# AniketRajpoot/DeepMusicGeneration

Measured on NVIDIA B200. Metric: generated_tokens_per_sec, higher is better.
Workload: dtype bf16

## Files before the change

deepmusicgeneration_b200/csrc/decode_layer.cu:

```cuda
#include <cuda.h>

#include "attention_decode3.cuh"
#include "kernels.cuh"
#include "launch.cuh"

namespace dmg {
namespace {

constexpr int DL_STAGES = 10;
constexpr int DL_STAGE = 128 * 128;
constexpr int DL_B_BYTES = DL_ROWS * 128;
constexpr int DL_D = 512;
constexpr int DL_XA_BYTES = DL_ROWS * DL_D * 2;
constexpr int DL_HS_KB = 4;
constexpr int DL_HS_BYTES = DL_HS_KB * DL_B_BYTES;
constexpr int DL_OWN = DL_ROWS / DL_CLUSTER;
constexpr int DL_X1_BYTES = DL_OWN * DL_D * 4;
constexpr int DL_MMAW = 2;
constexpr int DL_THREADS = 32 * (1 + DL_MMAW + 8);
constexpr int DL_EPI0 = 32 * (1 + DL_MMAW);
constexpr int DL_EPI = 256;
constexpr int DL_LN_BYTES = 4 * DL_D * 4;
constexpr int DL_SMEM = DL_STAGES * DL_STAGE + DL_XA_BYTES + DL_HS_BYTES + DL_X1_BYTES + DL_LN_BYTES + 512  + 1024 ;
constexpr int DL_TMEM_COLS = 512;
constexpr int DL_CHAIN = DL_ROWS;
static_assert(DL_SMEM <= 227 * 1024, "decode_layer_kernel: shared memory budget");

__device__ __forceinline__ uint64_t dl_desc_sw128(uint32_t smem_addr) {
  return (uint64_t)((smem_addr & 0x3FFFFu) >> 4) | (1ull << 16) | (64ull << 32) | (1ull << 46) | (2ull << 61);
}
__host__ __device__ constexpr uint32_t dl_idesc(int M, int N) {
  return (1u << 4) | (1u << 7) | (1u << 10) | ((uint32_t)(N >> 3) << 17) | ((uint32_t)(M >> 4) << 24);
}
__device__ __forceinline__ uint32_t dl_cluster_ctarank() {
  uint32_t r;
  asm volatile("mov.u32 %0, %%cluster_ctarank;" : "=r"(r));
  return r;
}
__device__ __forceinline__ void dl_arrive() { asm volatile("barrier.cluster.arrive.release;" ::: "memory"); }
__device__ __forceinline__ void dl_wait() { asm volatile("barrier.cluster.wait.acquire;" ::: "memory"); }
__device__ __forceinline__ void dl_fence_async_all() { asm volatile("fence.proxy.async;" ::: "memory"); }
__device__ __forceinline__ void dl_fence_async_smem() { asm volatile("fence.proxy.async.shared::cta;" ::: "memory"); }

__device__ __forceinline__ void tmem_ld_32x16(uint32_t taddr, uint32_t (&r)[16]) {
  asm volatile(
      "tcgen05.ld.sync.aligned.32x32b.x16.b32 {%0,%1,%2,%3,%4,%5,%6,%7,%8,%9,%10,%11,%12,%13,%14,%15}, [%16];"
      : "=r"(r[0]), "=r"(r[1]), "=r"(r[2]), "=r"(r[3]), "=r"(r[4]), "=r"(r[5]), "=r"(r[6]), "=r"(r[7]), "=r"(r[8]),
        "=r"(r[9]), "=r"(r[10]), "=r"(r[11]), "=r"(r[12]), "=r"(r[13]), "=r"(r[14]), "=r"(r[15])
      : "r"(taddr)
      : "memory");
}
__device__ __forceinline__ void dl_spin(uint64_t* bar, uint32_t parity) {
  uint32_t n = 0;
  while (!mbar_try_wait(bar, parity))
    if (++n > (1u << 27)) __trap();
}
__device__ __forceinline__ float4 ldcg4(const float* p) { return __ldcg((const float4*)p); }
__device__ __forceinline__ void dl_mark(unsigned long long* dbg, int role, int mark) {
  if (dbg == nullptr) return;
  unsigned long long t;
  asm volatile("mov.u64 %0, %%globaltimer;" : "=l"(t));
  dbg[role * 16 + mark] = t;
}

__device__ __forceinline__ float dl_gelu(float x) {
  float t;
  asm("tanh.approx.f32 %0, %1;" : "=f"(t) : "f"(0.7978845608028654f * (x + 0.044715f * x * x * x)));
  return 0.5f * x * (1.f + t);
}

__device__ __forceinline__ void dl_layernorm(float (&z)[64], const float* __restrict__ w, const float* __restrict__ b, int t) {
  float s = 0.f;
#pragma unroll
  for (int i = 0; i < 64; i++) s += z[i];
  s += __shfl_xor_sync(0xffffffffu, s, 1); s += __shfl_xor_sync(0xffffffffu, s, 2); s += __shfl_xor_sync(0xffffffffu, s, 4);
  const float mean = s * (1.f / DL_D);
  float q = 0.f;
#pragma unroll
  for (int i = 0; i < 64; i++) { const float c = z[i] - mean; q += c * c; }
  q += __shfl_xor_sync(0xffffffffu, q, 1); q += __shfl_xor_sync(0xffffffffu, q, 2); q += __shfl_xor_sync(0xffffffffu, q, 4);
  const float rstd = rsqrtf(q * (1.f / DL_D) + 1e-5f);
#pragma unroll
  for (int kb = 0; kb < 8; kb++) {
    const int c = 64 * kb + 8 * t;
    const float4 w0 = *(const float4*)(w + c), w1 = *(const float4*)(w + c + 4);
    const float4 b0 = *(const float4*)(b + c), b1 = *(const float4*)(b + c + 4);
    float* v = z + 8 * kb;
    v[0] = (v[0] - mean) * rstd * w0.x + b0.x; v[1] = (v[1] - mean) * rstd * w0.y + b0.y;
    v[2] = (v[2] - mean) * rstd * w0.z + b0.z; v[3] = (v[3] - mean) * rstd * w0.w + b0.w;
    v[4] = (v[4] - mean) * rstd * w1.x + b1.x; v[5] = (v[5] - mean) * rstd * w1.y + b1.y;
    v[6] = (v[6] - mean) * rstd * w1.z + b1.z; v[7] = (v[7] - mean) * rstd * w1.w + b1.w;
  }
}
__device__ __forceinline__ void dl_store_xa(uint8_t* xa_s, const float (&z)[64], int r, int t) {
#pragma unroll
  for (int kb = 0; kb < 8; kb++) {
    const float* v = z + 8 * kb;
    *(uint4*)(xa_s + kb * DL_B_BYTES + r * 128 + ((t ^ (r & 7)) << 4)) =
        make_uint4(pack_bf16x2(v[0], v[1]), pack_bf16x2(v[2], v[3]), pack_bf16x2(v[4], v[5]), pack_bf16x2(v[6], v[7]));
  }
}

__device__ __forceinline__ void dl_gather(uint32_t taddr, int nacc, float (&out)[16]) {
  uint32_t r[16];
  tmem_ld_32x16(taddr, r);
  tmem_ld_wait();
#pragma unroll
  for (int i = 0; i < 16; i++) out[i] = __uint_as_float(r[i]);
  for (int c = 1; c < nacc; c++) {
    tmem_ld_32x16(taddr + c * DL_CHAIN, r);
    tmem_ld_wait();
#pragma unroll
    for (int i = 0; i < 16; i++) out[i] += __uint_as_float(r[i]);
  }
}

__device__ __forceinline__ uint32_t dl_mapa(uint32_t local_addr, uint32_t rank) {
  uint32_t r;
  asm volatile("mapa.shared::cluster.u32 %0, %1, %2;" : "=r"(r) : "r"(local_addr), "r"(rank));
  return r;
}
__device__ __forceinline__ void dl_st_cluster_v4(uint32_t addr, uint4 v) {
  asm volatile("st.shared::cluster.v4.b32 [%0], {%1, %2, %3, %4};" ::"r"(addr), "r"(v.x), "r"(v.y), "r"(v.z), "r"(v.w) : "memory");
}

__device__ __forceinline__ void decode_layer_body(const CUtensorMap& tmAttn, const CUtensorMap& tmWo, const CUtensorMap& tmW1,
                                                  const CUtensorMap& tmW2, const CUtensorMap& tmWq, const DecodeLayerArgs& a_in, int cluster,
                                                  uint8_t* dl_smem) {
  DecodeLayerArgs a = a_in;
  if (cluster != 0 || dl_cluster_ctarank() != 0) a.dbg = nullptr;
  uint8_t* tiles = dl_smem + ((1024u - (smem_u32(dl_smem) & 1023u)) & 1023u);
  uint8_t* xa_s = tiles + DL_STAGES * DL_STAGE;
  uint8_t* hs_s = xa_s + DL_XA_BYTES;
  float* x1_s = (float*)(hs_s + DL_HS_BYTES);
  float* ln_s = x1_s + DL_OWN * DL_D;
  uint64_t* full = (uint64_t*)(ln_s + 4 * DL_D);
  uint64_t* empty = full + DL_STAGES;
  uint64_t* tmem_full = empty + DL_STAGES;
  uint64_t* xa_ready = tmem_full + 4;
  uint64_t* hs_ready = xa_ready + 2;
  uint64_t* attn_full = hs_ready + 1;
  uint32_t* tmem_holder = (uint32_t*)(attn_full + 1);

  const int warp = threadIdx.x >> 5, lane = threadIdx.x & 31;
  const int crank = (int)dl_cluster_ctarank();
  const int row0 = a.row_base + cluster * DL_ROWS;
  const bool body = (a.mode & 1) != 0, next = (a.mode & 2) != 0;
  const int nkb_A = a.HD >> 6, nkb_d = DL_D >> 6;
  constexpr int nB = 2, nC = 4, nD = 2;
  const int fB = a.di / DL_CLUSTER, fD = a.n3 / DL_CLUSTER;
  const int nA_use = body ? nkb_A : 0, nB_use = body ? nB * nkb_d : 0, nC_use = body ? nC * DL_HS_KB : 0, nD_use = next ? nD * nkb_d : 0;
  pdl_launch_dependents();

  if (warp == 0 && lane == 0) {
    tma_prefetch_desc(&tmWo); tma_prefetch_desc(&tmW1); tma_prefetch_desc(&tmW2); tma_prefetch_desc(&tmWq); tma_prefetch_desc(&tmAttn);
  }
  if (warp == 1 && lane == 0) {
    for (int s = 0; s < DL_STAGES; s++) { mbar_init(&full[s], 1); mbar_init(&empty[s], 1); }
    for (int p = 0; p < 4; p++) mbar_init(&tmem_full[p], DL_MMAW);
    mbar_init(&xa_ready[0], DL_EPI); mbar_init(&xa_ready[1], DL_EPI); mbar_init(hs_ready, DL_EPI); mbar_init(attn_full, 1);
    mbar_fence_init();
  }
  if (warp == 1 + DL_MMAW) tmem_alloc<DL_TMEM_COLS>(tmem_holder);
  tc_fence_before();
  __syncthreads();
  tc_fence_after();
  const uint32_t tmem_base = *tmem_holder;

  if (warp == 0) {
    if (lane == 0) dl_mark(a.dbg, 0, 0);
    const int total = nA_use + nB_use + nC_use + nD_use;
    int bar_state = 0;
    const uint64_t w_policy = l2_policy_evict_last();
    for (int r = 0; r < total; r += 8) {
      if (body && bar_state == 0 && r >= nA_use) { dl_arrive(); bar_state = 1; }
      if (body && bar_state == 1 && r + 8 > nA_use + DL_STAGES) { dl_wait(); dl_arrive(); bar_state = 2; }
      if (body && bar_state == 2 && r >= nA_use + nB_use) { dl_wait(); dl_arrive(); bar_state = 3; }
      if (body && bar_state == 3 && r + 8 > nA_use + nB_use + nC_use + DL_STAGES) { dl_wait(); dl_arrive(); bar_state = 4; }
      const int i = r + lane;
      if (lane < 8 && i < total) {
        const int s = i % DL_STAGES;
        if (i >= DL_STAGES) dl_spin(&empty[s], (uint32_t)((i / DL_STAGES) - 1) & 1u);
        uint8_t* dst = tiles + s * DL_STAGE;
        const CUtensorMap* tm; int c0, frow, boxes;
        if (i < nA_use) { tm = &tmWo; c0 = i * 64; frow = 64 * crank; boxes = 1; }
        else if (i < nA_use + nB_use) { const int j = i - nA_use; tm = &tmW1; c0 = (j / nB) * 64; frow = fB * crank + 128 * (j % nB); boxes = 2; }
        else if (i < nA_use + nB_use + nC_use) { const int j = i - nA_use - nB_use; tm = &tmW2; c0 = fB * crank + (j / nC) * 64; frow = 128 * (j % nC); boxes = 2; }
        else { const int j = i - nA_use - nB_use - nC_use; tm = &tmWq; c0 = (j / nD) * 64; frow = fD * crank + 128 * (j % nD); boxes = (j % nD) == 0 ? 2 : 1; }
        mbar_expect_tx(&full[s], (uint32_t)(boxes * 64 * 128));
        tma_load_2d_hint(dst, tm, c0, frow, &full[s], w_policy);
        if (boxes == 2) tma_load_2d_hint(dst + 64 * 128, tm, c0, frow + 64, &full[s], w_policy);
      }
      if (r == 0 && body) {
        pdl_wait();
        if (lane == 0) mbar_expect_tx(attn_full, (uint32_t)(nkb_A * DL_B_BYTES));
        __syncwarp();
        if (lane < nkb_A) tma_load_2d(xa_s + lane * DL_B_BYTES, &tmAttn, lane * 64, row0, attn_full);
      }
      __syncwarp();
    }
    if (lane == 0) dl_mark(a.dbg, 0, 6);
    if (body) {
      if (bar_state == 0) { dl_arrive(); bar_state = 1; }
      if (bar_state == 1) { dl_wait(); dl_arrive(); bar_state = 2; }
      if (bar_state == 2) { dl_wait(); dl_arrive(); bar_state = 3; }
      if (bar_state == 3) { dl_wait(); dl_arrive(); bar_state = 4; }
      dl_wait();
    }
  } else if (warp <= DL_MMAW) {
    int it = 0;
    const int mine = warp - 1;
    const uint32_t xa_addr = smem_u32(xa_s), hs_addr = smem_u32(hs_s), tiles_addr = smem_u32(tiles);
    constexpr uint64_t DHI = (1ull << 16) | (64ull << 32) | (1ull << 46) | (2ull << 61);
    auto kblock = [&](int i, uint32_t col, uint32_t idesc, uint32_t b_addr, int kb, int kbx) {
      if ((i & (DL_MMAW - 1)) != mine) return;
      const int s = i % DL_STAGES;
      dl_spin(&full[s], (uint32_t)(i / DL_STAGES) & 1u);
      tc_fence_after();
      if (elect_one()) {
        const uint64_t da = DHI | (uint64_t)(((tiles_addr + s * DL_STAGE) & 0x3FFFFu) >> 4), db = DHI | (uint64_t)((b_addr & 0x3FFFFu) >> 4);
        const uint32_t d = tmem_base + col + (uint32_t)(((kb & kbx) << 2) * DL_CHAIN);
#pragma unroll
        for (int l = 0; l < 4; l++)
          umma_bf16(d + (uint32_t)(l * DL_CHAIN), da + (uint64_t)(2 * l), db + (uint64_t)(2 * l), idesc, kb > kbx ? 1u : 0u);
        umma_commit(&empty[s]);
      }
      __syncwarp();
    };
    constexpr uint32_t ID64 = dl_idesc(64, DL_ROWS), ID128 = dl_idesc(128, DL_ROWS);
    if (lane == 0 && mine == 0) dl_mark(a.dbg, 1, 0);
    if (body) {
      {
        dl_spin(attn_full, 0);
        tc_fence_after();
        for (int kb = 0; kb < nkb_A; kb++) kblock(it++, 0, ID64, xa_addr + kb * DL_B_BYTES, kb, 1);
        if (elect_one()) {
          dl_mark(a.dbg, 1, 1);
          umma_commit(&tmem_full[0]);
        }
      }
      __syncwarp();
      dl_arrive();
      dl_wait();
      dl_arrive();
      {
        dl_spin(&xa_ready[0], 0);
        tc_fence_after();
        if (lane == 0) dl_mark(a.dbg, 1, 2);
        for (int kb = 0; kb < nkb_d; kb++)
          for (int t = 0; t < nB; t++) kblock(it++, (uint32_t)(t * 4 * DL_CHAIN), ID128, xa_addr + kb * DL_B_BYTES, kb, 0);
        if (elect_one()) {
          dl_mark(a.dbg, 1, 3);
          umma_commit(&tmem_full[1]);
        }
        __syncwarp();
        dl_spin(hs_ready, 0);
        tc_fence_after();
        for (int kb = 0; kb < DL_HS_KB; kb++)
          for (int t = 0; t < nC; t++) kblock(it++, (uint32_t)(t * 4 * DL_CHAIN), ID128, hs_addr + kb * DL_B_BYTES, kb, 0);
        if (elect_one()) {
          dl_mark(a.dbg, 1, 5);
          umma_commit(&tmem_full[2]);
        }
      }
      __syncwarp();
      dl_wait();
      dl_arrive();
      dl_wait();
      dl_arrive();
      dl_wait();
      asm volatile("fence.proxy.async.shared::cta;" ::: "memory");
    }
    if (next) {
      if (!body) dl_spin(&xa_ready[1], 0);
      tc_fence_after();
      if (lane == 0) dl_mark(a.dbg, 1, 6);
      for (int kb = 0; kb < nkb_d; kb++) {
        kblock(it++, 0, ID128, xa_addr + kb * DL_B_BYTES, kb, 0);
        kblock(it++, (uint32_t)(4 * DL_CHAIN), ID64, xa_addr + kb * DL_B_BYTES, kb, 0);
      }
      if (elect_one()) {
        dl_mark(a.dbg, 1, 7);
        umma_commit(&tmem_full[3]);
      }
    }
    __syncwarp();
  } else {
    const int q = warp & 3;
    const int half = (warp - 1 - DL_MMAW) >> 2;
    const int te = threadIdx.x - DL_EPI0;
    const int r = te >> 3, t = te & 7;
    const int lr = te >> 6, lc = te & 63;
    const int row = row0 + r;
    const bool valid = row < a.B;
    const int erow0 = row0 + 16 * half;
    const uint32_t tq = tmem_base + ((uint32_t)(q * 32) << 16) + (uint32_t)(16 * half);
    float z[64];
    const bool mk = te == 0;
    if (body) {
      const float* src[4] = {a.ln1w, a.ln1b, a.ln2w, a.ln2b};
#pragma unroll
      for (int i = 0; i < 4; i++) *(float2*)(ln_s + i * DL_D + 2 * te) = __ldg((const float2*)(src[i] + 2 * te));
      asm volatile("bar.sync 1, 256;" ::: "memory");
    }
    if (mk) dl_mark(a.dbg, 2, 0);
    pdl_wait();
    if (mk) dl_mark(a.dbg, 2, 1);
    float rs[8] = {0.f, 0.f, 0.f, 0.f, 0.f, 0.f, 0.f, 0.f};
    if (body) {
      if (valid) {
        const float4 x0 = ldcg4(a.x32 + (size_t)row * DL_D + 64 * crank + 8 * t), x1 = ldcg4(a.x32 + (size_t)row * DL_D + 64 * crank + 8 * t + 4);
        rs[0] = x0.x; rs[1] = x0.y; rs[2] = x0.z; rs[3] = x0.w; rs[4] = x1.x; rs[5] = x1.y; rs[6] = x1.z; rs[7] = x1.w;
      }
    } else {
#pragma unroll
      for (int kb = 0; kb < 8; kb++) {
        float4 x0 = make_float4(0.f, 0.f, 0.f, 0.f), x1 = x0;
        if (valid) { x0 = ldcg4(a.x32 + (size_t)row * DL_D + 64 * kb + 8 * t); x1 = ldcg4(a.x32 + (size_t)row * DL_D + 64 * kb + 8 * t + 4); }
        float* v = z + 8 * kb;
        v[0] = x0.x; v[1] = x0.y; v[2] = x0.z; v[3] = x0.w; v[4] = x1.x; v[5] = x1.y; v[6] = x1.z; v[7] = x1.w;
      }
    }
    float acc[16];
    if (body) {
      mbar_wait(&tmem_full[0], 0);
      tc_fence_after();
      if (mk) dl_mark(a.dbg, 2, 2);
      dl_gather(tq, 4 * nkb_A < 8 ? 4 * nkb_A : 8, acc);
      float* T = (float*)hs_s;
      float4* stats = (float4*)(hs_s + DL_ROWS * 64 * 4);
      if (lane < 16) {
        const int fl = 16 * q + lane;
        const float bias = a.bo ? __ldg(a.bo + 64 * crank + fl) : 0.f;
#pragma unroll
        for (int rr = 0; rr < 16; rr++) T[(16 * half + rr) * 64 + fl] = acc[rr] + bias;
      }
      tc_fence_before();
      asm volatile("bar.sync 1, 256;" ::: "memory");
      if (mk) dl_mark(a.dbg, 2, 3);
      float v[8];
      {
        const float4 t0 = *(const float4*)(T + r * 64 + 8 * t), t1 = *(const float4*)(T + r * 64 + 8 * t + 4);
        v[0] = t0.x + rs[0]; v[1] = t0.y + rs[1]; v[2] = t0.z + rs[2]; v[3] = t0.w + rs[3];
        v[4] = t1.x + rs[4]; v[5] = t1.y + rs[5]; v[6] = t1.z + rs[6]; v[7] = t1.w + rs[7];
      }
      float s1 = 0.f;
#pragma unroll
      for (int i = 0; i < 8; i++) s1 += v[i];
      s1 += __shfl_xor_sync(0xffffffffu, s1, 1); s1 += __shfl_xor_sync(0xffffffffu, s1, 2); s1 += __shfl_xor_sync(0xffffffffu, s1, 4);
      const float mj = s1 * (1.f / 64.f);
      float s2 = 0.f;
#pragma unroll
      for (int i = 0; i < 8; i++) { const float c = v[i] - mj; s2 += c * c; }
      s2 += __shfl_xor_sync(0xffffffffu, s2, 1); s2 += __shfl_xor_sync(0xffffffffu, s2, 2); s2 += __shfl_xor_sync(0xffffffffu, s2, 4);
      {
        const uint32_t off = smem_u32(stats + crank * DL_ROWS + r);
        dl_st_cluster_v4(dl_mapa(off, (uint32_t)t), make_uint4(__float_as_uint(mj), __float_as_uint(s2), 0u, 0u));
      }
      dl_arrive();
      dl_wait();
      if (mk) dl_mark(a.dbg, 2, 4);
      {
        float ms[DL_CLUSTER], qs[DL_CLUSTER], mean = 0.f;
#pragma unroll
        for (int p = 0; p < DL_CLUSTER; p++) { const float4 st = stats[p * DL_ROWS + r]; ms[p] = st.x; qs[p] = st.y; mean += st.x; }
        mean *= (1.f / DL_CLUSTER);
        float m2 = 0.f;
#pragma unroll
        for (int p = 0; p < DL_CLUSTER; p++) { const float dm = ms[p] - mean; m2 += qs[p] + 64.f * dm * dm; }
        const float rstd = rsqrtf(m2 * (1.f / DL_D) + 1e-5f);
        const float* w = ln_s + 64 * crank + 8 * t;
        const float* bb = ln_s + DL_D + 64 * crank + 8 * t;
#pragma unroll
        for (int i = 0; i < 8; i++) v[i] = (v[i] - mean) * rstd * w[i] + bb[i];
      }
      {
        const uint32_t xoff = smem_u32(x1_s + (r & 3) * DL_D + 64 * crank + 8 * t);
        const uint32_t xo = dl_mapa(xoff, (uint32_t)(r >> 2));
        dl_st_cluster_v4(xo, make_uint4(__float_as_uint(v[0]), __float_as_uint(v[1]), __float_as_uint(v[2]), __float_as_uint(v[3])));
        dl_st_cluster_v4(xo + 16, make_uint4(__float_as_uint(v[4]), __float_as_uint(v[5]), __float_as_uint(v[6]), __float_as_uint(v[7])));
        const uint4 packed = make_uint4(pack_bf16x2(v[0], v[1]), pack_bf16x2(v[2], v[3]), pack_bf16x2(v[4], v[5]), pack_bf16x2(v[6], v[7]));
        const uint32_t off = smem_u32(xa_s) + (uint32_t)(crank * DL_B_BYTES + r * 128 + ((t ^ (r & 7)) << 4));
#pragma unroll
        for (int p = 0; p < DL_CLUSTER; p++) dl_st_cluster_v4(dl_mapa(off, (uint32_t)p), packed);
      }
      dl_arrive();
      dl_wait();
      asm volatile("fence.proxy.async.shared::cta;" ::: "memory");
      mbar_arrive(&xa_ready[0]);
      if (mk) dl_mark(a.dbg, 2, 5);
      mbar_wait(&tmem_full[1], 0);
      tc_fence_after();
      if (mk) dl_mark(a.dbg, 2, 6);
#pragma unroll
      for (int tt = 0; tt < nB; tt++) {
        dl_gather(tq + tt * 4 * DL_CHAIN, 4, acc);
        const int fl = 128 * tt + 32 * q + lane;
        const float bias = a.b1 ? __ldg(a.b1 + fB * crank + fl) : 0.f;
        uint8_t* base = hs_s + (fl >> 6) * DL_B_BYTES + (fl & 7) * 2;
        const int ch = (fl & 63) >> 3;
#pragma unroll
        for (int rr = 0; rr < 16; rr++) {
          const int rw = 16 * half + rr;
          *(bf16*)(base + rw * 128 + ((ch ^ (rw & 7)) << 4)) = __float2bfloat16_rn(dl_gelu(acc[rr] + bias));
        }
      }
      tc_fence_before();
      dl_fence_async_smem();
      mbar_arrive(hs_ready);
      if (mk) dl_mark(a.dbg, 2, 7);
      mbar_wait(&tmem_full[2], 0);
      tc_fence_after();
      if (mk) dl_mark(a.dbg, 2, 9);
      float* pp = a.PP + (size_t)crank * a.pp_stride;
#pragma unroll
      for (int tt = 0; tt < nC; tt++) {
        dl_gather(tq + tt * 4 * DL_CHAIN, 4, acc);
        const int f = 128 * tt + 32 * q + lane;
#pragma unroll
        for (int rr = 0; rr < 16; rr++) pp[(size_t)(erow0 + rr) * DL_D + f] = acc[rr];
      }
      tc_fence_before();
      __syncwarp();
      if (mk) dl_mark(a.dbg, 2, 10);
      dl_arrive();
      dl_wait();
      if (mk) dl_mark(a.dbg, 2, 11);
      {
        const int crow = DL_OWN * crank + lr;
        const int grow = row0 + crow;
        const int c0 = 8 * lc;
        float v[8];
        const float4 xa0 = *(const float4*)(x1_s + lr * DL_D + c0), xa1 = *(const float4*)(x1_s + lr * DL_D + c0 + 4);
        v[0] = xa0.x; v[1] = xa0.y; v[2] = xa0.z; v[3] = xa0.w; v[4] = xa1.x; v[5] = xa1.y; v[6] = xa1.z; v[7] = xa1.w;
        if (a.b2) {
          const float4 b0 = __ldg((const float4*)(a.b2 + c0)), b1 = __ldg((const float4*)(a.b2 + c0 + 4));
          v[0] += b0.x; v[1] += b0.y; v[2] += b0.z; v[3] += b0.w; v[4] += b1.x; v[5] += b1.y; v[6] += b1.z; v[7] += b1.w;
        }
#pragma unroll
        for (int p = 0; p < DL_CLUSTER; p++) {
          const float* src = a.PP + (size_t)p * a.pp_stride + (size_t)grow * DL_D + c0;
          const float4 p0 = ldcg4(src), p1 = ldcg4(src + 4);
          v[0] += p0.x; v[1] += p0.y; v[2] += p0.z; v[3] += p0.w; v[4] += p1.x; v[5] += p1.y; v[6] += p1.z; v[7] += p1.w;
        }
        float* red = (float*)(tmem_holder + 4);
        float s1 = 0.f;
#pragma unroll
        for (int i = 0; i < 8; i++) s1 += v[i];
        s1 = warp_sum(s1);
        if (lane == 0) red[(te >> 5)] = s1;
        asm volatile("bar.sync 1, 256;" ::: "memory");
        const float mean = (red[2 * lr] + red[2 * lr + 1]) * (1.f / DL_D);
        float s2 = 0.f;
#pragma unroll
        for (int i = 0; i < 8; i++) { const float c = v[i] - mean; s2 += c * c; }
        s2 = warp_sum(s2);
        if (lane == 0) red[8 + (te >> 5)] = s2;
        asm volatile("bar.sync 1, 256;" ::: "memory");
        const float rstd = rsqrtf((red[8 + 2 * lr] + red[8 + 2 * lr + 1]) * (1.f / DL_D) + 1e-5f);
        const float* w = ln_s + 2 * DL_D + c0;
        const float* bb = ln_s + 3 * DL_D + c0;
#pragma unroll
        for (int i = 0; i < 8; i++) v[i] = (v[i] - mean) * rstd * w[i] + bb[i];
        const uint4 packed = make_uint4(pack_bf16x2(v[0], v[1]), pack_bf16x2(v[2], v[3]), pack_bf16x2(v[4], v[5]), pack_bf16x2(v[6], v[7]));
        if (grow < a.B) {
          float* dst = a.x32 + (size_t)grow * DL_D + c0;
          *(float4*)dst = make_float4(v[0], v[1], v[2], v[3]);
          *(float4*)(dst + 4) = make_float4(v[4], v[5], v[6], v[7]);
          if (a.xa_out) *(uint4*)(a.xa_out + (size_t)grow * DL_D + c0) = packed;
        }
        if (next) {
          const uint32_t off = smem_u32(xa_s) + (uint32_t)((lc >> 3) * DL_B_BYTES + crow * 128 + (((lc & 7) ^ (crow & 7)) << 4));
#pragma unroll
          for (int p = 0; p < DL_CLUSTER; p++) dl_st_cluster_v4(dl_mapa(off, (uint32_t)p), packed);
        }
      }
      if (mk) dl_mark(a.dbg, 2, 12);
      dl_arrive();
      dl_wait();
    } else if (next) {
      dl_store_xa(xa_s, z, r, t);
      dl_fence_async_smem();
      mbar_arrive(&xa_ready[1]);
    }
    if (next) {
      mbar_wait(&tmem_full[3], 0);
      tc_fence_after();
      if (mk) dl_mark(a.dbg, 2, 13);
#pragma unroll
      for (int tt = 0; tt < nD; tt++) {
        dl_gather(tq + tt * 4 * DL_CHAIN, 4, acc);
        const bool h64 = tt == 1;
        const int f = fD * crank + (h64 ? 128 + 16 * q + lane : 32 * q + lane);
        if (!h64 || lane < 16) {
          const float bias = a.bq ? __ldg(a.bq + f) : 0.f;
#pragma unroll
          for (int rr = 0; rr < 16; rr++)
            if (erow0 + rr < a.B) a.qkv[(size_t)(erow0 + rr) * a.n3 + f] = acc[rr] + bias;
        }
      }
      tc_fence_before();
      if (mk) dl_mark(a.dbg, 2, 14);
    }
  }
  __syncthreads();
  if (warp == 1 + DL_MMAW) tmem_dealloc<DL_TMEM_COLS>(tmem_base);
}

__global__ void __launch_bounds__(DL_THREADS, 1)
decode_layer_kernel(const __grid_constant__ CUtensorMap tmAttn, const __grid_constant__ CUtensorMap tmWo,
                    const __grid_constant__ CUtensorMap tmW1, const __grid_constant__ CUtensorMap tmW2,
                    const __grid_constant__ CUtensorMap tmWq, const DecodeLayerArgs a) {
  extern __shared__ __align__(1024) uint8_t dyn_smem[];
  decode_layer_body(tmAttn, tmWo, tmW1, tmW2, tmWq, a, (int)blockIdx.x / DL_CLUSTER, dyn_smem);
}

static_assert(D3_THREADS <= DL_THREADS, "the attention role runs on the first D3_THREADS threads of the block");
__global__ void __launch_bounds__(DL_THREADS, 1)
decode_dual_kernel(const __grid_constant__ CUtensorMap tmAttn, const __grid_constant__ CUtensorMap tmWo,
                   const __grid_constant__ CUtensorMap tmW1, const __grid_constant__ CUtensorMap tmW2,
                   const __grid_constant__ CUtensorMap tmWq, const DecodeLayerArgs fa, const __grid_constant__ CUtensorMap tmK,
                   const __grid_constant__ CUtensorMap tmV, const __grid_constant__ CUtensorMap tmR, const AttnDecodeArgs aa, int n_stages,
                   int b0, int n_fused) {
  extern __shared__ __align__(1024) uint8_t dyn_smem[];
  const int cluster = (int)blockIdx.x / DL_CLUSTER;
  if (cluster < n_fused) {
    decode_layer_body(tmAttn, tmWo, tmW1, tmW2, tmWq, fa, cluster, dyn_smem);
  } else if (threadIdx.x < D3_THREADS) {
    attn_decode3_body<D3_TEAMS>(tmK, tmV, tmR, aa, n_stages, b0, (int)blockIdx.x - n_fused * DL_CLUSTER,
                                (int)gridDim.x - n_fused * DL_CLUSTER, dyn_smem);
  }
}

}

bool decode_layer_supported(int d, int HD, int di, int n3) {
  return d == DL_D && HD % 64 == 0 && HD >= 64 && HD <= DL_D && di == DL_CLUSTER * 64 * DL_HS_KB && n3 == DL_CLUSTER * 192;
}

int decode_layer(const TensorMap2D* tmAttn, const TensorMap2D* tmWo, const TensorMap2D* tmW1, const TensorMap2D* tmW2,
                 const TensorMap2D* tmWq, const DecodeLayerArgs& a, cudaStream_t st) {
  DMG_CHECK(decode_layer_supported(a.d, a.HD, a.di, a.n3), "decode_layer: geometry d=%d HD=%d di=%d n3=%d not supported", a.d, a.HD, a.di, a.n3);
  static bool configured = false;
  if (!configured) {
    DMG_CUDA_OK(cudaFuncSetAttribute(decode_layer_kernel, cudaFuncAttributeMaxDynamicSharedMemorySize, DL_SMEM));
    configured = true;
  }
  const int clusters = (a.B - a.row_base + DL_ROWS - 1) / DL_ROWS;
  if (clusters <= 0) return 0;
  return launch_k(decode_layer_kernel, dim3(clusters * DL_CLUSTER), dim3(DL_THREADS), (size_t)DL_SMEM, st, DL_CLUSTER,
                  *(const CUtensorMap*)tmAttn->bytes, *(const CUtensorMap*)tmWo->bytes, *(const CUtensorMap*)tmW1->bytes,
                  *(const CUtensorMap*)tmW2->bytes, *(const CUtensorMap*)tmWq->bytes, a);
}


bool decode_dual_supported(int M) { return attn_decode3_supported(64, M); }
int decode_dual_max_items(int attn_clusters) { return attn_clusters * DL_CLUSTER * D3_CAP; }

int decode_dual_max_clusters() {
  static int cached = -1;
  if (cached >= 0) return cached;
  cudaLaunchConfig_t cfg = {};
  cfg.gridDim = dim3(DL_CLUSTER * 32); cfg.blockDim = dim3(DL_THREADS); cfg.dynamicSmemBytes = 227 * 1024;
  cudaLaunchAttribute attr[1];
  attr[0].id = cudaLaunchAttributeClusterDimension;
  attr[0].val.clusterDim.x = DL_CLUSTER; attr[0].val.clusterDim.y = 1; attr[0].val.clusterDim.z = 1;
  cfg.attrs = attr; cfg.numAttrs = 1;
  int n = 0;
  if (cudaFuncSetAttribute(decode_dual_kernel, cudaFuncAttributeMaxDynamicSharedMemorySize, 227 * 1024) != cudaSuccess ||
      cudaOccupancyMaxActiveClusters(&n, decode_dual_kernel, &cfg) != cudaSuccess) {
    cudaGetLastError();
    n = 0;
  }
  cached = n;
  return cached;
}

int decode_dual(const TensorMap2D* tmAttn, const TensorMap2D* tmWo, const TensorMap2D* tmW1, const TensorMap2D* tmW2, const TensorMap2D* tmWq,
                const DecodeLayerArgs& fa, const TensorMap2D* tmK, const TensorMap2D* tmV, const TensorMap2D* tmR, const AttnDecodeArgs& aa,
                int b0, int attn_clusters, cudaStream_t st) {
  DMG_CHECK(decode_layer_supported(fa.d, fa.HD, fa.di, fa.n3) && decode_dual_supported(aa.M), "decode_dual: geometry not supported");
  DMG_CHECK(aa.Dcap >= aa.M + 1, "decode_dual: rel-pos cache too small (%d < %d)", aa.Dcap, aa.M + 1);
  DMG_CHECK((long long)aa.B * aa.H <= decode_dual_max_items(attn_clusters), "decode_dual: %d x %d items do not fit %d attention clusters",
            aa.B, aa.H, attn_clusters);
  const int ns = d3_pick_stages(aa.M);
  const D3Layout L = d3_layout(aa.M, ns);
  const int smem = L.total > DL_SMEM ? L.total : DL_SMEM;
  static int configured = 0;
  if (configured < smem) {
    DMG_CUDA_OK(cudaFuncSetAttribute(decode_dual_kernel, cudaFuncAttributeMaxDynamicSharedMemorySize, smem));
    configured = smem;
  }
  const int n_fused = (fa.B - fa.row_base + DL_ROWS - 1) / DL_ROWS;
  DMG_CHECK(n_fused >= 1 && attn_clusters >= 1, "decode_dual: empty role");
  return launch_k(decode_dual_kernel, dim3((n_fused + attn_clusters) * DL_CLUSTER), dim3(DL_THREADS), (size_t)smem, st, DL_CLUSTER,
                  *(const CUtensorMap*)tmAttn->bytes, *(const CUtensorMap*)tmWo->bytes, *(const CUtensorMap*)tmW1->bytes,
                  *(const CUtensorMap*)tmW2->bytes, *(const CUtensorMap*)tmWq->bytes, fa, *(const CUtensorMap*)tmK->bytes,
                  *(const CUtensorMap*)tmV->bytes, *(const CUtensorMap*)tmR->bytes, aa, ns, b0, n_fused);
}

}
```

deepmusicgeneration_b200/csrc/sampling.cu:

```cuda
#include "kernels.cuh"
#include "sampling.cuh"
#include "launch.cuh"

namespace dmg {

__device__ __forceinline__ uint32_t mulhilo(uint32_t a, uint32_t b, uint32_t* hi) {
  const uint64_t p = (uint64_t)a * b;
  *hi = (uint32_t)(p >> 32);
  return (uint32_t)p;
}
__device__ float philox_uniform(uint64_t seed, uint64_t offset, uint32_t stream) {
  uint32_t c0 = (uint32_t)offset, c1 = (uint32_t)(offset >> 32), c2 = stream, c3 = 0x9E3779B9u;
  uint32_t k0 = (uint32_t)seed, k1 = (uint32_t)(seed >> 32);
#pragma unroll
  for (int i = 0; i < 10; i++) {
    uint32_t hi0, hi1;
    const uint32_t lo0 = mulhilo(0xD2511F53u, c0, &hi0);
    const uint32_t lo1 = mulhilo(0xCD9E8D57u, c2, &hi1);
    c0 = hi1 ^ c1 ^ k0;
    c1 = lo1;
    c2 = hi0 ^ c3 ^ k1;
    c3 = lo0;
    k0 += 0x9E3779B9u;
    k1 += 0xBB67AE85u;
  }
  return (float)(c0 >> 8) * (1.0f / 16777216.0f);
}

__device__ __forceinline__ uint32_t float_key(float f) {
  const uint32_t u = __float_as_uint(f);
  return (u & 0x80000000u) ? ~u : (u | 0x80000000u);
}
__device__ __forceinline__ float key_float(uint32_t k) {
  const uint32_t u = (k & 0x80000000u) ? (k & 0x7fffffffu) : ~k;
  return __uint_as_float(u);
}

constexpr int SAMP_THREADS = 256;
constexpr int SAMP_MAXV = 1024;

__device__ void warp0_inclusive_scan(float* vals, int n) {
  if (threadIdx.x >= 32) return;
  const int lane = threadIdx.x;
  float carry = 0.f;
  for (int base = 0; base < n; base += 32) {
    const int i = base + lane;
    float x = i < n ? vals[i] : 0.f;
#pragma unroll
    for (int o = 1; o < 32; o <<= 1) {
      const float y = __shfl_up_sync(0xffffffffu, x, o);
      if (lane >= o) x += y;
    }
    x += carry;
    if (i < n) vals[i] = x;
    carry = __shfl_sync(0xffffffffu, x, 31);
  }
}

__device__ float block_max(float v, float* scratch) {
  v = warp_max(v);
  __syncthreads();
  if ((threadIdx.x & 31) == 0) scratch[threadIdx.x >> 5] = v;
  __syncthreads();
  float r = scratch[0];
  for (int w = 1; w < SAMP_THREADS / 32; w++) r = fmaxf(r, scratch[w]);
  return r;
}
__device__ float block_sum(float v, float* scratch) {
  v = warp_sum(v);
  __syncthreads();
  if ((threadIdx.x & 31) == 0) scratch[threadIdx.x >> 5] = v;
  __syncthreads();
  float r = 0.f;
  for (int w = 0; w < SAMP_THREADS / 32; w++) r += scratch[w];
  return r;
}

__device__ __forceinline__ bool in_range(int x, int lo, int hi) { return x >= lo && x < hi; }

__global__ void __launch_bounds__(SAMP_THREADS) sample_kernel(SampleArgs a) {
  __shared__ float l[SAMP_MAXV];
  __shared__ unsigned long long keys[SAMP_MAXV];
  __shared__ unsigned long long kin[SAMP_MAXV];
  __shared__ float pr[SAMP_MAXV];
  __shared__ float scratch[SAMP_THREADS / 32];
  __shared__ int sh_int[4];

  const int sidx = blockIdx.x, tid = threadIdx.x;
  pdl_launch_dependents();
  pdl_wait();
  const int V = a.V;
  const dmg_vocab_layout vl = a.vocab;
  const dmg_sampler_params sp = a.params;
  const float NEG = -INFINITY;

  int prev, repeat_count, last_xxsep = 0, status = 0, step = 0;
  long long last_pos = 0, start_pos = 0;
  if (a.loop_mode == 2) {
    prev = a.prev_idx[sidx];
    repeat_count = a.repeat_count[sidx];
    last_xxsep = a.last_xxsep[sidx];
    last_pos = a.last_pos[sidx];
  } else if (a.loop_mode) {
    status = a.status[sidx];
    prev = a.prev_idx[sidx];
    repeat_count = a.repeat_count[sidx];
    last_xxsep = a.last_xxsep[sidx];
    last_pos = a.last_pos[sidx];
    start_pos = a.start_pos[sidx];
    step = a.step[sidx];
    if (status != 0) {
      if (tid == 0) {
        if (a.out_tokens) a.out_tokens[sidx] = status == 1 ? -1 : -2;
        a.next_ids[sidx] = vl.pad;
        if (a.next_pos) a.next_pos[sidx] = last_pos;
      }
      return;
    }
  } else {
    prev = a.prev_idx[sidx];
    repeat_count = a.repeat_count[sidx];
  }
  const bool prev_dur = in_range(prev, vl.dur_lo, vl.dur_hi);
  const bool prev_note = prev == vl.sep || in_range(prev, vl.note_lo, vl.note_hi);
  const bool prev_ins = prev == vl.ni || in_range(prev, vl.ins_lo, vl.ins_hi);
  const bool remix = (sp.flags & DMG_SAMPLE_REMIX_FILTER) != 0;

  double temperature;
  if (a.loop_mode) {
    if (prev == vl.sep) last_xxsep = 1;
    else if (prev_ins && prev == vl.ni) last_xxsep = 0;
    if (prev_dur) temperature = sp.temperatures[2];
    else if (prev_note) temperature = sp.temperatures[1];
    else if (prev_ins || prev == vl.pad) temperature = sp.temperatures[0];
    else {
      if (tid == 0) {
        if (a.out_tokens) a.out_tokens[sidx] = -2;
        if (a.loop_mode == 1) {
          a.status[sidx] = 2;
          a.next_ids[sidx] = vl.pad;
          if (a.next_pos) a.next_pos[sidx] = last_pos;
        }
      }
      return;
    }
  } else {
    temperature = (prev == vl.pad || prev_dur) ? sp.temperatures[0] : sp.temperatures[1];
  }
  {
    double pen = log(((double)repeat_count + 1.0) / 4.0) / 5.0;
    if (pen < 0.0) pen = 0.0;
    temperature += pen * temperature;
  }
  const float tf = (float)temperature;
  const bool forbid_bos = a.loop_mode && (((last_pos - start_pos) / 16) <= (long long)sp.min_bars);

  const float* lg = a.logits + (size_t)sidx * V;
  for (int i = tid; i < V; i += SAMP_THREADS) {
    float x = lg[i];
    if (temperature != 1.0) x = x / tf;
    bool kill = false;
    const bool is_special = in_range(i, vl.special_lo, vl.special_hi);
    const bool is_note = in_range(i, vl.note_lo, vl.note_hi);
    const bool is_dur = in_range(i, vl.dur_lo, vl.dur_hi);
    const bool is_ins = in_range(i, vl.ins_lo, vl.ins_hi);
    if (forbid_bos && i == vl.bos) kill = true;
    if (!a.loop_mode) {
      if (is_special && i != vl.pad && i != vl.mask) kill = true;
    }
    if (sp.allowed_ins_mask != 0 && is_ins && !((sp.allowed_ins_mask >> (i - vl.ins_lo)) & 1u)) kill = true;
    if (last_xxsep) { if (is_ins) kill = true; }
    else if (i == vl.ni) kill = true;
    if (remix && prev == vl.pad) {
      if (is_dur || is_ins || (is_special && i != vl.sep)) kill = true;
    } else if (prev_dur) {
      if (is_dur || is_note || (is_special && i != vl.ni)) kill = true;
    } else if (prev_ins || (!remix && prev == vl.pad)) {
      if (is_ins || is_dur || (is_special && i != vl.sep)) kill = true;
    } else {
      if (is_note || is_ins || is_special) kill = true;
    }
    if ((sp.flags & DMG_SAMPLE_MASK_UNUSED) && i >= vl.ins_hi) kill = true;
    l[i] = kill ? NEG : x;
  }
  __syncthreads();

  for (int i = tid; i < V; i += SAMP_THREADS)
    kin[i] = ((unsigned long long)float_key(l[i]) << 32) | (unsigned long long)(0xFFFFFFFFu - (uint32_t)i);
  __syncthreads();
  for (int i = tid; i < V; i += SAMP_THREADS) {
    const unsigned long long me = kin[i];
    int r = 0;
#pragma unroll 4
    for (int j = 0; j < V; j++) r += kin[j] > me ? 1 : 0;
    keys[r] = me;
  }
  __syncthreads();

  int top_k = sp.top_k < V ? sp.top_k : V;
  float kth = NEG;
  if (top_k > 0) {
    kth = key_float((uint32_t)(keys[top_k - 1] >> 32));
    for (int i = tid; i < V; i += SAMP_THREADS)
      if (l[i] < kth) l[i] = NEG;
  }
  __syncthreads();

  if (sp.top_p > 0.0f) {
    const float smax = key_float((uint32_t)(keys[0] >> 32));
    float part = 0.f;
    for (int i = tid; i < V; i += SAMP_THREADS) {
      float x = key_float((uint32_t)(keys[i] >> 32));
      if (top_k > 0 && x < kth) x = NEG;
      const float e = (smax == NEG) ? 0.f : expf(x - smax);
      pr[i] = e;
      part += e;
    }
    const float tot = block_sum(part, scratch);
    for (int i = tid; i < V; i += SAMP_THREADS) pr[i] = pr[i] / tot;
    __syncthreads();
    warp0_inclusive_scan(pr, V);
    __syncthreads();
    for (int i = tid + 1; i < V; i += SAMP_THREADS) {
      if (pr[i - 1] > sp.top_p) {
        const int idx = (int)(0xFFFFFFFFu - (uint32_t)(keys[i] & 0xFFFFFFFFull));
        l[idx] = NEG;
      }
    }
    __syncthreads();
  }

  float part = NEG;
  for (int i = tid; i < V; i += SAMP_THREADS) part = fmaxf(part, l[i]);
  const float mx = block_max(part, scratch);
  float ps = 0.f;
  for (int i = tid; i < V; i += SAMP_THREADS) {
    const float e = (mx == NEG) ? 0.f : expf(l[i] - mx);
    pr[i] = e;
    ps += e;
  }
  const float tot = block_sum(ps, scratch);
  int nz = 0;
  for (int i = tid; i < V; i += SAMP_THREADS) {
    const float p = pr[i] / tot;
    pr[i] = p;
    if (a.probs) a.probs[(size_t)sidx * V + i] = p;
    nz += p > 0.f ? 1 : 0;
  }
  const int num_choices = (int)(block_sum((float)nz, scratch) + 0.5f);
  __syncthreads();
  warp0_inclusive_scan(pr, V);
  __syncthreads();
  if (tid == 0) sh_int[0] = V;
  __syncthreads();
  const uint64_t draw = a.offset + (a.loop_mode ? (uint64_t)step : 0ull) + (a.dev_offset ? (uint64_t)*a.dev_offset : 0ull);
  const float u = philox_uniform(sp.seed, draw, a.stream_ids ? (uint32_t)a.stream_ids[sidx] : (uint32_t)sidx);
  const float target = u * pr[V - 1];
  for (int i = tid; i < V; i += SAMP_THREADS) {
    const float prevc = i > 0 ? pr[i - 1] : 0.f;
    if (pr[i] > target && pr[i] > prevc) atomicMin(&sh_int[0], i);
  }
  __syncthreads();
  int idx = sh_int[0];
  if (idx >= V) {
    __syncthreads();
    if (tid == 0) sh_int[1] = -1;
    __syncthreads();
    for (int i = tid; i < V; i += SAMP_THREADS) {
      const float prevc = i > 0 ? pr[i - 1] : 0.f;
      if (pr[i] > prevc) atomicMax(&sh_int[1], i);
    }
    __syncthreads();
    idx = sh_int[1] >= 0 ? sh_int[1] : vl.pad;
  }

  if (tid != 0) return;
  if (a.num_choices) a.num_choices[sidx] = num_choices;
  if (a.loop_mode != 1) {
    a.out_tokens[sidx] = idx;
    return;
  }
  if (num_choices <= 2) repeat_count += 1;
  else repeat_count = repeat_count / 2;
  bool stop = false;
  if (prev == vl.sep) {
    last_pos += (long long)(idx - vl.dur_lo);
    const long long abs_bar = last_pos / 16;
    if ((sp.flags & DMG_SAMPLE_EARLY_STOP) && ((double)step / (double)sp.n_words > 0.80) && (abs_bar % 4 == 0)) stop = true;
  }
  if (!stop && (sp.flags & DMG_SAMPLE_EARLY_STOP) && idx == vl.bos) stop = true;
  a.repeat_count[sidx] = repeat_count;
  a.last_xxsep[sidx] = last_xxsep;
  a.last_pos[sidx] = last_pos;
  a.step[sidx] = step + 1;
  if (stop) {
    a.status[sidx] = 1;
    if (a.out_tokens) a.out_tokens[sidx] = -1;
    a.next_ids[sidx] = vl.pad;
  } else {
    a.prev_idx[sidx] = idx;
    if (a.out_tokens) a.out_tokens[sidx] = idx;
    a.next_ids[sidx] = idx;
  }
  if (a.next_pos) a.next_pos[sidx] = last_pos;
}

__device__ void block_arg_best(float v, int idx, bool want_max, float* sval, int* sidx, float& best_v, int& best_i) {
  for (int o = 16; o > 0; o >>= 1) {
    const float ov = __shfl_xor_sync(0xffffffffu, v, o);
    const int oi = __shfl_xor_sync(0xffffffffu, idx, o);
    const bool better = want_max ? (ov > v || (ov == v && oi < idx)) : (ov < v || (ov == v && oi < idx));
    if (better) { v = ov; idx = oi; }
  }
  __syncthreads();
  if ((threadIdx.x & 31) == 0) { sval[threadIdx.x >> 5] = v; sidx[threadIdx.x >> 5] = idx; }
  __syncthreads();
  best_v = sval[0]; best_i = sidx[0];
  for (int w = 1; w < SAMP_THREADS / 32; w++) {
    const float ov = sval[w]; const int oi = sidx[w];
    const bool better = want_max ? (ov > best_v || (ov == best_v && oi < best_i)) : (ov < best_v || (ov == best_v && oi < best_i));
    if (better) { best_v = ov; best_i = oi; }
  }
}

__global__ void __launch_bounds__(SAMP_THREADS) beam_step_kernel(BeamArgs a) {
  __shared__ float lp[SAMP_MAXV];
  __shared__ float cand_score[SAMP_MAXV];
  __shared__ int cand_tok[SAMP_MAXV];
  __shared__ float scratch[SAMP_THREADS / 32];
  __shared__ float sval[SAMP_THREADS / 32];
  __shared__ int sidx[SAMP_THREADS / 32];
  const int tid = threadIdx.x, V = a.V, K = a.top_k;
  const float INF = INFINITY;
  pdl_launch_dependents();
  pdl_wait();
  for (int row = 0; row < a.nb; row++) {
    const float* lg = a.logits + (size_t)row * V;
    float part = -INF;
    for (int i = tid; i < V; i += SAMP_THREADS) { lp[i] = lg[i]; part = fmaxf(part, lg[i]); }
    const float mx = block_max(part, scratch);
    float ps = 0.f;
    for (int i = tid; i < V; i += SAMP_THREADS) ps += expf(lp[i] - mx);
    const float lse = mx + logf(block_sum(ps, scratch));
    __syncthreads();
    for (int i = tid; i < V; i += SAMP_THREADS) lp[i] -= lse;
    __syncthreads();
    const float prev = a.scores_in[a.n_scores == 1 ? 0 : row];
    for (int j = 0; j < K; j++) {
      float v = -INF; int idx = 0x7fffffff;
      for (int i = tid; i < V; i += SAMP_THREADS)
        if (lp[i] > v || (lp[i] == v && i < idx)) { v = lp[i]; idx = i; }
      float bv; int bi;
      block_arg_best(v, idx, true, sval, sidx, bv, bi);
      if (tid == 0) { cand_score[row * K + j] = -bv + prev; cand_tok[row * K + j] = bi; lp[bi] = -INF; }
      __syncthreads();
    }
  }
  const int NC = a.nb * K;
  for (int j = 0; j < a.beam_sz; j++) {
    float v = INF; int idx = 0x7fffffff;
    for (int i = tid; i < NC; i += SAMP_THREADS)
      if (cand_score[i] < v || (cand_score[i] == v && i < idx)) { v = cand_score[i]; idx = i; }
    float bv; int bi;
    block_arg_best(v, idx, false, sval, sidx, bv, bi);
    if (tid == 0) {
      if (j < NC) { a.scores_out[j] = bv; a.parents[j] = bi / K; a.tokens[j] = cand_tok[bi]; cand_score[bi] = INF; }
    }
    __syncthreads();
  }
}

int beam_step_launch(const BeamArgs& a, cudaStream_t st) {
  DMG_CHECK(a.V <= SAMP_MAXV && a.nb >= 1 && a.top_k >= 1 && a.top_k <= a.V && a.nb * a.top_k <= SAMP_MAXV && a.beam_sz >= 1 &&
                a.beam_sz <= a.nb * a.top_k,
            "beam step: nb %d x top_k %d (beam_sz %d, vocab %d) outside the kernel's limits", a.nb, a.top_k, a.beam_sz, a.V);
  return launch_k(beam_step_kernel, dim3(1), dim3(SAMP_THREADS), 0, st, 1, a);
}

int sample_launch(const SampleArgs& a, int n, cudaStream_t st) {
  DMG_CHECK(a.V <= SAMP_MAXV, "sampler: vocab %d exceeds %d", a.V, SAMP_MAXV);
  if (n <= 0) return 0;
  return launch_k(sample_kernel, dim3(n), dim3(SAMP_THREADS), 0, st, 1, a);
}

}
```

Measured before the change: 289,400.

## Replace cluster barriers with st.async mbarrier pushes and speed up sampling sort/scan

Result: faster. 297,300, median of 6 (+2.7%).

```diff
diff --git a/deepmusicgeneration_b200/csrc/decode_layer.cu b/deepmusicgeneration_b200/csrc/decode_layer.cu
--- a/deepmusicgeneration_b200/csrc/decode_layer.cu
+++ b/deepmusicgeneration_b200/csrc/decode_layer.cu
@@ -22,6 +22,11 @@
 constexpr int DL_EPI = 256;
 constexpr int DL_LN_BYTES = 4 * DL_D * 4;
 constexpr int DL_SMEM = DL_STAGES * DL_STAGE + DL_XA_BYTES + DL_HS_BYTES + DL_X1_BYTES + DL_LN_BYTES + 512  + 1024 ;
+constexpr int DL_T_BYTES = DL_ROWS * 64 * 4;
+constexpr int DL_STATS_TX = DL_CLUSTER * DL_ROWS * 16;
+constexpr int DL_LN1_TX = DL_CLUSTER * (DL_B_BYTES + DL_OWN * 64 * 4);
+static_assert(DL_T_BYTES + DL_STATS_TX <= DL_HS_BYTES, "slice statistics land in HS behind the out-projection slice");
+static_assert(DL_LN1_TX == DL_XA_BYTES + DL_X1_BYTES, "LayerNorm-1 exchange: XA filled by 8 k-blocks, X1 by 8 slices");
 constexpr int DL_TMEM_COLS = 512;
 constexpr int DL_CHAIN = DL_ROWS;
 static_assert(DL_SMEM <= 227 * 1024, "decode_layer_kernel: shared memory budget");
@@ -39,7 +44,6 @@
 }
 __device__ __forceinline__ void dl_arrive() { asm volatile("barrier.cluster.arrive.release;" ::: "memory"); }
 __device__ __forceinline__ void dl_wait() { asm volatile("barrier.cluster.wait.acquire;" ::: "memory"); }
-__device__ __forceinline__ void dl_fence_async_all() { asm volatile("fence.proxy.async;" ::: "memory"); }
 __device__ __forceinline__ void dl_fence_async_smem() { asm volatile("fence.proxy.async.shared::cta;" ::: "memory"); }
 
 __device__ __forceinline__ void tmem_ld_32x16(uint32_t taddr, uint32_t (&r)[16]) {
@@ -54,6 +58,19 @@
   uint32_t n = 0;
   while (!mbar_try_wait(bar, parity))
     if (++n > (1u << 27)) __trap();
+}
+__device__ __forceinline__ void dl_spin_peers(uint64_t* bar) {
+  uint32_t n = 0, ok = 0;
+  while (!ok) {
+    asm volatile(
+        "{\n\t.reg .pred p;\n\t"
+        "mbarrier.try_wait.parity.acquire.cluster.shared::cta.b64 p, [%1], 0;\n\t"
+        "selp.u32 %0, 1, 0, p;\n\t}"
+        : "=r"(ok)
+        : "r"(smem_u32(bar))
+        : "memory");
+    if (++n > (1u << 27)) __trap();
+  }
 }
 __device__ __forceinline__ float4 ldcg4(const float* p) { return __ldcg((const float4*)p); }
 __device__ __forceinline__ void dl_mark(unsigned long long* dbg, int role, int mark) {
@@ -119,6 +136,14 @@
   uint32_t r;
   asm volatile("mapa.shared::cluster.u32 %0, %1, %2;" : "=r"(r) : "r"(local_addr), "r"(rank));
   return r;
+}
+__device__ __forceinline__ void dl_push(uint32_t local_addr, uint4 v, uint64_t* local_bar, uint32_t rank) {
+  asm volatile("st.async.shared::cluster.mbarrier::complete_tx::bytes.v4.b32 [%0], {%1, %2, %3, %4}, [%5];"
+               ::"r"(dl_mapa(local_addr, rank)), "r"(v.x), "r"(v.y), "r"(v.z), "r"(v.w), "r"(dl_mapa(smem_u32(local_bar), rank))
+               : "memory");
+}
+__device__ __forceinline__ void dl_push(uint32_t local_addr, float4 v, uint64_t* local_bar, uint32_t rank) {
+  dl_push(local_addr, make_uint4(__float_as_uint(v.x), __float_as_uint(v.y), __float_as_uint(v.z), __float_as_uint(v.w)), local_bar, rank);
 }
 __device__ __forceinline__ void dl_st_cluster_v4(uint32_t addr, uint4 v) {
   asm volatile("st.shared::cluster.v4.b32 [%0], {%1, %2, %3, %4};" ::"r"(addr), "r"(v.x), "r"(v.y), "r"(v.z), "r"(v.w) : "memory");
@@ -140,7 +165,8 @@
   uint64_t* xa_ready = tmem_full + 4;
   uint64_t* hs_ready = xa_ready + 2;
   uint64_t* attn_full = hs_ready + 1;
-  uint32_t* tmem_holder = (uint32_t*)(attn_full + 1);
+  uint64_t* stats_full = attn_full + 1;
+  uint32_t* tmem_holder = (uint32_t*)(stats_full + 1);
 
   const int warp = threadIdx.x >> 5, lane = threadIdx.x & 31;
   const int crank = (int)dl_cluster_ctarank();
@@ -158,7 +184,10 @@
   if (warp == 1 && lane == 0) {
     for (int s = 0; s < DL_STAGES; s++) { mbar_init(&full[s], 1); mbar_init(&empty[s], 1); }
     for (int p = 0; p < 4; p++) mbar_init(&tmem_full[p], DL_MMAW);
-    mbar_init(&xa_ready[0], DL_EPI); mbar_init(&xa_ready[1], DL_EPI); mbar_init(hs_ready, DL_EPI); mbar_init(attn_full, 1);
+    mbar_init(hs_ready, DL_EPI); mbar_init(attn_full, 1);
+    mbar_init(stats_full, 1); mbar_expect_tx(stats_full, DL_STATS_TX);
+    mbar_init(&xa_ready[0], 1); mbar_expect_tx(&xa_ready[0], DL_LN1_TX);
+    mbar_init(&xa_ready[1], DL_EPI);
     mbar_fence_init();
   }
   if (warp == 1 + DL_MMAW) tmem_alloc<DL_TMEM_COLS>(tmem_holder);
@@ -166,6 +195,7 @@
   __syncthreads();
   tc_fence_after();
   const uint32_t tmem_base = *tmem_holder;
+  if (body) dl_arrive();
 
   if (warp == 0) {
     if (lane == 0) dl_mark(a.dbg, 0, 0);
@@ -173,10 +203,8 @@
     int bar_state = 0;
     const uint64_t w_policy = l2_policy_evict_last();
     for (int r = 0; r < total; r += 8) {
-      if (body && bar_state == 0 && r >= nA_use) { dl_arrive(); bar_state = 1; }
-      if (body && bar_state == 1 && r + 8 > nA_use + DL_STAGES) { dl_wait(); dl_arrive(); bar_state = 2; }
-      if (body && bar_state == 2 && r >= nA_use + nB_use) { dl_wait(); dl_arrive(); bar_state = 3; }
-      if (body && bar_state == 3 && r + 8 > nA_use + nB_use + nC_use + DL_STAGES) { dl_wait(); dl_arrive(); bar_state = 4; }
+      if (body && bar_state == 0 && r >= nA_use + nB_use) { dl_wait(); dl_arrive(); bar_state = 1; }
+      if (body && bar_state == 1 && r + 8 > nA_use + nB_use + nC_use + DL_STAGES) { dl_wait(); dl_arrive(); bar_state = 2; }
       const int i = r + lane;
       if (lane < 8 && i < total) {
         const int s = i % DL_STAGES;
@@ -201,10 +229,8 @@
     }
     if (lane == 0) dl_mark(a.dbg, 0, 6);
     if (body) {
-      if (bar_state == 0) { dl_arrive(); bar_state = 1; }
+      if (bar_state == 0) { dl_wait(); dl_arrive(); bar_state = 1; }
       if (bar_state == 1) { dl_wait(); dl_arrive(); bar_state = 2; }
-      if (bar_state == 2) { dl_wait(); dl_arrive(); bar_state = 3; }
-      if (bar_state == 3) { dl_wait(); dl_arrive(); bar_state = 4; }
       dl_wait();
     }
   } else if (warp <= DL_MMAW) {
@@ -240,11 +266,9 @@
         }
       }
       __syncwarp();
-      dl_arrive();
-      dl_wait();
-      dl_arrive();
       {
-        dl_spin(&xa_ready[0], 0);
+        dl_spin_peers(&xa_ready[0]);
+        dl_fence_async_smem();
         tc_fence_after();
         if (lane == 0) dl_mark(a.dbg, 1, 2);
         for (int kb = 0; kb < nkb_d; kb++)
@@ -269,7 +293,7 @@
       dl_wait();
       dl_arrive();
       dl_wait();
-      asm volatile("fence.proxy.async.shared::cta;" ::: "memory");
+      dl_fence_async_smem();
     }
     if (next) {
       if (!body) dl_spin(&xa_ready[1], 0);
@@ -353,12 +377,9 @@
 #pragma unroll
       for (int i = 0; i < 8; i++) { const float c = v[i] - mj; s2 += c * c; }
       s2 += __shfl_xor_sync(0xffffffffu, s2, 1); s2 += __shfl_xor_sync(0xffffffffu, s2, 2); s2 += __shfl_xor_sync(0xffffffffu, s2, 4);
-      {
-        const uint32_t off = smem_u32(stats + crank * DL_ROWS + r);
-        dl_st_cluster_v4(dl_mapa(off, (uint32_t)t), make_uint4(__float_as_uint(mj), __float_as_uint(s2), 0u, 0u));
-      }
-      dl_arrive();
       dl_wait();
+      dl_push(smem_u32(stats + crank * DL_ROWS + r), make_uint4(__float_as_uint(mj), __float_as_uint(s2), 0u, 0u), stats_full, (uint32_t)t);
+      dl_spin_peers(stats_full);
       if (mk) dl_mark(a.dbg, 2, 4);
       {
         float ms[DL_CLUSTER], qs[DL_CLUSTER], mean = 0.f;
@@ -376,18 +397,13 @@
       }
       {
         const uint32_t xoff = smem_u32(x1_s + (r & 3) * DL_D + 64 * crank + 8 * t);
-        const uint32_t xo = dl_mapa(xoff, (uint32_t)(r >> 2));
-        dl_st_cluster_v4(xo, make_uint4(__float_as_uint(v[0]), __float_as_uint(v[1]), __float_as_uint(v[2]), __float_as_uint(v[3])));
-        dl_st_cluster_v4(xo + 16, make_uint4(__float_as_uint(v[4]), __float_as_uint(v[5]), __float_as_uint(v[6]), __float_as_uint(v[7])));
+        dl_push(xoff, make_float4(v[0], v[1], v[2], v[3]), &xa_ready[0], (uint32_t)(r >> 2));
+        dl_push(xoff + 16, make_float4(v[4], v[5], v[6], v[7]), &xa_ready[0], (uint32_t)(r >> 2));
         const uint4 packed = make_uint4(pack_bf16x2(v[0], v[1]), pack_bf16x2(v[2], v[3]), pack_bf16x2(v[4], v[5]), pack_bf16x2(v[6], v[7]));
         const uint32_t off = smem_u32(xa_s) + (uint32_t)(crank * DL_B_BYTES + r * 128 + ((t ^ (r & 7)) << 4));
 #pragma unroll
-        for (int p = 0; p < DL_CLUSTER; p++) dl_st_cluster_v4(dl_mapa(off, (uint32_t)p), packed);
-      }
-      dl_arrive();
-      dl_wait();
-      asm volatile("fence.proxy.async.shared::cta;" ::: "memory");
-      mbar_arrive(&xa_ready[0]);
+        for (int p = 0; p < DL_CLUSTER; p++) dl_push(off, packed, &xa_ready[0], (uint32_t)p);
+      }
       if (mk) dl_mark(a.dbg, 2, 5);
       mbar_wait(&tmem_full[1], 0);
       tc_fence_after();
@@ -431,6 +447,7 @@
         const int grow = row0 + crow;
         const int c0 = 8 * lc;
         float v[8];
+        dl_spin_peers(&xa_ready[0]);
         const float4 xa0 = *(const float4*)(x1_s + lr * DL_D + c0), xa1 = *(const float4*)(x1_s + lr * DL_D + c0 + 4);
         v[0] = xa0.x; v[1] = xa0.y; v[2] = xa0.z; v[3] = xa0.w; v[4] = xa1.x; v[5] = xa1.y; v[6] = xa1.z; v[7] = xa1.w;
         if (a.b2) {
diff --git a/deepmusicgeneration_b200/csrc/sampling.cu b/deepmusicgeneration_b200/csrc/sampling.cu
--- a/deepmusicgeneration_b200/csrc/sampling.cu
+++ b/deepmusicgeneration_b200/csrc/sampling.cu
@@ -39,21 +39,35 @@
 constexpr int SAMP_THREADS = 256;
 constexpr int SAMP_MAXV = 1024;
 
-__device__ void warp0_inclusive_scan(float* vals, int n) {
-  if (threadIdx.x >= 32) return;
-  const int lane = threadIdx.x;
-  float carry = 0.f;
-  for (int base = 0; base < n; base += 32) {
-    const int i = base + lane;
-    float x = i < n ? vals[i] : 0.f;
-#pragma unroll
-    for (int o = 1; o < 32; o <<= 1) {
-      const float y = __shfl_up_sync(0xffffffffu, x, o);
-      if (lane >= o) x += y;
-    }
-    x += carry;
-    if (i < n) vals[i] = x;
-    carry = __shfl_sync(0xffffffffu, x, 31);
+__device__ void block_inclusive_scan(float* vals, int n, float* carry) {
+  constexpr int NW = SAMP_THREADS / 32, PER_WARP = SAMP_MAXV / 32 / NW;
+  const int lane = threadIdx.x & 31, w = threadIdx.x >> 5, nch = (n + 31) >> 5;
+  float loc[PER_WARP];
+#pragma unroll
+  for (int k = 0; k < PER_WARP; k++) {
+    const int c = w + NW * k;
+    if (c < nch) {
+      const int i = 32 * c + lane;
+      float x = i < n ? vals[i] : 0.f;
+#pragma unroll
+      for (int o = 1; o < 32; o <<= 1) {
+        const float y = __shfl_up_sync(0xffffffffu, x, o);
+        if (lane >= o) x += y;
+      }
+      loc[k] = x;
+      if (lane == 31) carry[c] = x;
+    }
+  }
+  __syncthreads();
+  if (threadIdx.x == 0) {
+    float cy = 0.f;
+    for (int c = 0; c < nch; c++) { const float t = carry[c]; carry[c] = cy; cy = t + cy; }
+  }
+  __syncthreads();
+#pragma unroll
+  for (int k = 0; k < PER_WARP; k++) {
+    const int c = w + NW * k, i = 32 * c + lane;
+    if (c < nch && i < n) vals[i] = loc[k] + carry[c];
   }
 }
 
@@ -83,10 +97,13 @@
   __shared__ unsigned long long keys[SAMP_MAXV];
   __shared__ unsigned long long kin[SAMP_MAXV];
   __shared__ float pr[SAMP_MAXV];
+  __shared__ unsigned long long gk[SAMP_MAXV];
   __shared__ float scratch[SAMP_THREADS / 32];
+  __shared__ float carry[SAMP_MAXV / 32];
+  __shared__ int low_count[SAMP_MAXV / 32];
   __shared__ int sh_int[4];
 
-  const int sidx = blockIdx.x, tid = threadIdx.x;
+  const int sidx = blockIdx.x, tid = threadIdx.x, lane = tid & 31, warp = tid >> 5;
   pdl_launch_dependents();
   pdl_wait();
   const int V = a.V;
@@ -155,6 +172,7 @@
   const float tf = (float)temperature;
   const bool forbid_bos = a.loop_mode && (((last_pos - start_pos) / 16) <= (long long)sp.min_bars);
 
+  if (tid == 0) { sh_int[2] = 0; sh_int[3] = 0; }
   const float* lg = a.logits + (size_t)sidx * V;
   for (int i = tid; i < V; i += SAMP_THREADS) {
     float x = lg[i];
@@ -185,15 +203,52 @@
   }
   __syncthreads();
 
-  for (int i = tid; i < V; i += SAMP_THREADS)
-    kin[i] = ((unsigned long long)float_key(l[i]) << 32) | (unsigned long long)(0xFFFFFFFFu - (uint32_t)i);
-  __syncthreads();
-  for (int i = tid; i < V; i += SAMP_THREADS) {
-    const unsigned long long me = kin[i];
-    int r = 0;
+  const uint32_t key_neg = float_key(NEG);
+  const int nchunk = (V + SAMP_THREADS - 1) / SAMP_THREADS;
+  uint32_t low_ballot[SAMP_MAXV / SAMP_THREADS];
+#pragma unroll
+  for (int c = 0; c < SAMP_MAXV / SAMP_THREADS; c++) {
+    if (c >= nchunk) break;
+    const int i = tid + c * SAMP_THREADS;
+    bool low = false;
+    if (i < V) {
+      const uint32_t fk = float_key(l[i]);
+      const unsigned long long k = ((unsigned long long)fk << 32) | (unsigned long long)(0xFFFFFFFFu - (uint32_t)i);
+      kin[i] = k;
+      if (fk > key_neg) gk[atomicAdd(&sh_int[2], 1)] = k;
+      else { low = true; if (fk < key_neg) sh_int[3] = 1; }
+    }
+    low_ballot[c] = __ballot_sync(0xffffffffu, low);
+    if (lane == 0) low_count[c * (SAMP_THREADS / 32) + warp] = __popc(low_ballot[c]);
+  }
+  __syncthreads();
+  if (sh_int[3]) {
+    for (int i = tid; i < V; i += SAMP_THREADS) {
+      const unsigned long long me = kin[i];
+      int r = 0;
 #pragma unroll 4
-    for (int j = 0; j < V; j++) r += kin[j] > me ? 1 : 0;
-    keys[r] = me;
+      for (int j = 0; j < V; j++) r += kin[j] > me ? 1 : 0;
+      keys[r] = me;
+    }
+  } else {
+    const int n_hi = sh_int[2];
+    for (int s = tid; s < n_hi; s += SAMP_THREADS) {
+      const unsigned long long me = gk[s];
+      int r = 0;
+#pragma unroll 4
+      for (int j = 0; j < n_hi; j++) r += gk[j] > me ? 1 : 0;
+      keys[r] = me;
+    }
+#pragma unroll
+    for (int c = 0; c < SAMP_MAXV / SAMP_THREADS; c++) {
+      if (c >= nchunk) break;
+      const int i = tid + c * SAMP_THREADS;
+      if (i < V && ((low_ballot[c] >> lane) & 1u)) {
+        int r = n_hi + __popc(low_ballot[c] & ((1u << lane) - 1u));
+        for (int e = 0; e < c * (SAMP_THREADS / 32) + warp; e++) r += low_count[e];
+        keys[r] = kin[i];
+      }
+    }
   }
   __syncthreads();
 
@@ -219,7 +274,7 @@
     const float tot = block_sum(part, scratch);
     for (int i = tid; i < V; i += SAMP_THREADS) pr[i] = pr[i] / tot;
     __syncthreads();
-    warp0_inclusive_scan(pr, V);
+    block_inclusive_scan(pr, V, carry);
     __syncthreads();
     for (int i = tid + 1; i < V; i += SAMP_THREADS) {
       if (pr[i - 1] > sp.top_p) {
@@ -249,7 +304,7 @@
   }
   const int num_choices = (int)(block_sum((float)nz, scratch) + 0.5f);
   __syncthreads();
-  warp0_inclusive_scan(pr, V);
+  block_inclusive_scan(pr, V, carry);
   __syncthreads();
   if (tid == 0) sh_int[0] = V;
   __syncthreads();
```
